# nschloe/flow

Hardware: AMD Instinct MI355X
Metric: ipcs_time_steps_per_sec (higher is better)
Workload: dtype f64

## Files before the change

flow_amd/_hip.py:

```python
import ctypes
import os

import torch

from . import device

_HERE = os.path.dirname(os.path.abspath(__file__))
LIB_PATH = os.path.join(_HERE, 'csrc', 'libflow_hip.so')

REDUCE_WORK = 4096
GMRES_MAX_RESTART = 30
GMRES_PARTIALS = (GMRES_MAX_RESTART + 2) * 1024
GMRES_STATE = 1280
SPMV_ROWS_PER_BLOCK = 256
SPMV_NNZ_PER_BLOCK = 1022
PMG_NNZ_PER_BLOCK = 2044

c_double_p = ctypes.c_void_p
c_int_p = ctypes.c_void_p


class Operator(ctypes.Structure):
    _fields_ = [
        ('kind', ctypes.c_int),
# ... 270 lines not shown

class MomentumJvp(ctypes.Structure):
    _fields_ = [
        ('mesh', ctypes.POINTER(MeshS)),
        ('W', ctypes.POINTER(SpaceS)),
        ('bfmask', ctypes.c_void_p),
        ('ui', ctypes.c_void_p),
        ('prm', NsParams),
        ('scratch', ctypes.c_void_p),
        ('nbc', ctypes.c_int),
        ('bc_dofs', ctypes.c_void_p),
        ('bc_mask', ctypes.c_void_p),
        ]


_VP = ctypes.c_void_p
_I = ctypes.c_int
_D = ctypes.c_double
_P = ctypes.POINTER
SYMBOLS = {
    'flow_abi_version': [],
    'flow_launch_count': [_P(ctypes.c_ulonglong)],
    'flow_graph_mode': [_I, ctypes.c_longlong],
    'flow_graph_stats': [_P(ctypes.c_ulonglong)],
    'flow_xcd_tile_host': [_I, _I],
    'flow_spmv_tile_nnz': [_I],
    'flow_operator_apply': [_P(Operator), _VP, _VP, _VP],
    'flow_profile_spmv_begin': [_I, _I],
    'flow_profile_spmv_end': [_P(_D), _P(_I)],
    'flow_profile_event_overhead': [_P(_D), _VP],
    'flow_profile_marker': [_I, _VP],
    'flow_profile_stream_copy': [ctypes.c_size_t, _VP, _VP, _VP],
    'flow_profile_stream_read': [ctypes.c_size_t, _VP, _VP, _VP],
    'flow_operator_diag_inv': [_P(Operator), _VP, _VP, _VP],
    'flow_dot_host': [_I, _VP, _VP, _VP, _P(_D), _VP],
    'flow_norm_host': [_I, _VP, _I, _VP, _P(_D), _VP],
    'flow_axpby': [_I, _D, _VP, _D, _VP, _VP],
    'flow_vmul': [_I, _D, _VP, _VP, _VP, _VP],
    'flow_fill': [_I, _D, _VP, _VP],
    'flow_lincomb': [_I, _I, _P(_D), _P(_VP), _VP, _VP],
    'flow_fingerprint': [_I, _P(_VP), _P(_I), _VP, _VP, _VP],
    'flow_read_doubles': [_VP, _I, _P(_D), _VP],
    'flow_extrapolation_weights': [_I, _P(_D), _D, _I, _I, _P(_D)],
    'flow_scale_rows': [_I, _VP, _VP, _VP, _VP],
    'flow_cg_solve': [_P(Operator), _VP, _P(CoarseS), _P(MgS), _VP, _VP, _D, _D,
                      _I, _I, _I, _VP, ctypes.c_size_t, _P(_I), _P(_D), _VP],
# ... 259 lines not shown
```

flow_amd/csrc/common.h:

```cpp
#pragma once
#include <hip/hip_runtime.h>

#include <algorithm>
#include <cstdarg>
#include <cstdio>
#include <functional>
#include <vector>

#include "../../include/flow_hip.h"

namespace flow {
extern unsigned long long g_launches;
}
#undef hipLaunchKernelGGL
#define hipLaunchKernelGGL(kernelName, numBlocks, numThreads, memPerBlock,        \
                           streamId, ...)                                       \
  do {                                                                          \
    ++flow::g_launches;                                                         \
    (kernelName)<<<(numBlocks), (numThreads), (memPerBlock), (streamId)>>>(     \
        __VA_ARGS__);                                                           \
  } while (0)

namespace flow {

// ... 6 lines not shown
int ilu_check(const flow_ilu* ilu, int op_size);

int pmg_apply(const flow_pmg* M, const double* r, double* z, hipStream_t st,
              const double* stop = nullptr);
int pmg_check(const flow_pmg* M, int op_size);
int tl_apply(const flow_tl* T, const double* r, double* z, hipStream_t st,
             const double* stop = nullptr);
int tl_check(const flow_tl* T, int op_size);
int operator_apply(const flow_operator* A, const double* x, double* y,
                   hipStream_t st, const double* stop = nullptr);
int operator_size(const flow_operator* A);
int sum_partials_host(double* work, int nparts, double* host, hipStream_t st);
int check_operator(const flow_operator* A);
int fill(int n, double value, double* y, hipStream_t st);
struct NoEarly {
  __device__ __forceinline__ void operator()(int, bool) const {}
};

enum Slot {
  kGamma = 0, kAlpha, kBeta, kRes2, kB2, kRho, kOmega, kRhoNew, kTmp,
  kBreak, kTarget2, kDone, kConvIt, kIter, kNumSlots = 16
};
int read_state(const double* S, double* host, hipStream_t st);
int check_comm(const flow_comm* c, long long need);
int check_rows(const flow_rows* R);
int exchange(const flow_comm* c, int count);
int exchange_halo(const flow_comm* C, const flow_rows* R, int ncomp, int sum_count,
                  int hoff, hipStream_t st);

int gather(int nout, int nplanes, const int* ptr, const int* src,
           const double* scratch, size_t plane_stride, double* out,
           hipStream_t st, size_t out_stride = 0, int r0 = 0, int r1 = 0,
           const double* stop = nullptr, const unsigned char* idrow = nullptr,
           const double* v = nullptr, size_t v_stride = 0);
int momentum_jvp_check(const flow_momentum_jvp* J);
int momentum_jvp_apply(const flow_momentum_jvp* J, const double* v, double* out,
                       hipStream_t st, int v_stride = 0, int out_stride = 0,
                       const double* stop = nullptr,
                       const double* prm_dev = nullptr);
int momentum_jvp_params(const flow_momentum_jvp* J, double* dst, hipStream_t st);

constexpr long long kReplayAutoRows = 1500000;
struct KeyHash {
  unsigned long long h = 1469598103934665603ull;
  void bytes(const void* p, size_t n) {
    const unsigned char* c = static_cast<const unsigned char*>(p);
// ... 119 lines not shown
```

flow_amd/csrc/la_kernels.hip:

```cpp
#include <cstring>

#include "common.h"
#include "csr_stream.h"

namespace flow {

thread_local char g_error[512] = "";

void set_error(const char* fmt, ...) {
  va_list ap;
  va_start(ap, fmt);
  vsnprintf(g_error, sizeof(g_error), fmt, ap);
  va_end(ap);
}

static_assert(3 * kRedBlocks + kNumSlots <= FLOW_REDUCE_WORK, "work size");


template <bool DOT>
__global__ __launch_bounds__(kBlock) void spmv_stream_kernel(
    int n, const int* __restrict__ rowptr, const int* __restrict__ cols,
    const double* __restrict__ vals0, const double* __restrict__ vals1,
    const int* __restrict__ rowblocks, const double* __restrict__ x,
    double* __restrict__ y, double* __restrict__ dpart,
// ... 1116 lines not shown
    if (state[kDone] == 1.0) {
      *iters_host = static_cast<int>(state[kConvIt]);
      *resid_host = sqrt(res2);
      return FLOW_OK;
    }
    if (launched >= maxit) {
      *iters_host = launched;
      *resid_host = sqrt(res2);
      set_error("BiCGStab did not converge in %d iterations: |r| = %.3e > %.3e",
                launched, sqrt(res2), sqrt(state[kTarget2]));
      return FLOW_NOT_CONVERGED;
    }
  }
}

}

using namespace flow;

extern "C" const char* flow_last_error(void) { return g_error; }
extern "C" int flow_abi_version(void) { return 30; }

namespace flow {
unsigned long long g_launches = 0;
}
extern "C" int flow_launch_count(unsigned long long* count_host) {
  FLOW_REQUIRE(count_host != nullptr, "flow_launch_count argument");
  *count_host = flow::g_launches;
  return FLOW_OK;
}

extern "C" int flow_spmv_tile_nnz(int kind) {
  return (kind == 2 || kind == 4) ? kTile2 - 2 : kTile - 2;
}

extern "C" int flow_xcd_tile_host(int block, int nblocks) {
  return xcd_tile(block, nblocks);
}

extern "C" int flow_profile_spmv_begin(int rows, int max_launches) {
  SpmvProfile& pf = g_spmv_profile;
  FLOW_REQUIRE(rows > 0 && max_launches > 0 && max_launches <= 100000,
               "profile arguments");
  FLOW_REQUIRE(pf.ev == nullptr, "a profile is already running");
  pf.ev = new hipEvent_t[2 * static_cast<size_t>(max_launches)];
  for (int i = 0; i < 2 * max_launches; ++i)
// ... 729 lines not shown
  const double snj = dj > 0.0 ? et / dj : 0.0;
  const double resid = fabs(snj * g[j]);
  store_scalar(S + kRes2, resid);
  store_scalar(S + kConvIt, static_cast<double>(j + 1));
  const bool done = resid <= target && !lucky;
  if (done || lucky || last) {
    const int nc = j + 1;
    col[j] = dj;
    g[j] = csj * g[j];
    for (int i = nc - 1; i >= 0; --i) {
      double t = g[i];
      for (int c = i + 1; c < nc; ++c) t -= Hs[c * ld + i] * y[c];
      const double rii = Hs[i * ld + i];
      y[i] = rii != 0.0 ? t / rii : 0.0;
    }
    for (int k = 0; k < nc; ++k) store_scalar(G + kGYc + k, y[k] / nrm[k]);
    if (done) store_scalar(S + kDone, 1.0);
    if (lucky) store_scalar(S + kDone, 3.0);
  }
}

__global__ __launch_bounds__(kBlock) void gmres_begin_kernel(
    int nparts, int have_b2, int first, int accept10, double rtol, double atol,
    const double* __restrict__ partial, double* __restrict__ S) {
  double r = 0.0, b = 0.0;
  for (int i = threadIdx.x; i < nparts; i += kBlock) {
    r += load_scalar(partial + i);
    if (have_b2) b += load_scalar(partial + kRedBlocks + i);
  }
  r = block_sum(r);
  b = block_sum(b);
  if (threadIdx.x != 0) return;
  double target;
  if (first) {
    const double b2 = have_b2 ? b : r;
    target = fmax(rtol * sqrt(b2), atol);
    store_scalar(S + kB2, b2);
    store_scalar(S + kTarget2, target);
    if (have_b2 && r > b2) {
      store_scalar(S + kTmp, 1.0);
      r = b2;
    }
  } else {
    target = load_scalar(S + kTarget2);
  }
  const double beta = sqrt(r);
  store_scalar(S + kBeta, beta);
  store_scalar(S + kRes2, beta);
  store_scalar(S + kConvIt, 0.0);
  if (!(r == r))
    store_scalar(S + kDone, 2.0);
  else if (beta <= target || (accept10 && beta <= 10.0 * target))
    store_scalar(S + kDone, 4.0);
}

// ... 143 lines not shown
  hipLaunchKernelGGL(gmres_dots_kernel<NV>, dim3(gd), dim3(kBlock), 0, st, N,  \
                     w, V + static_cast<size_t>(k0) * N,                      \
                     static_cast<size_t>(N), k0 == 0 ? 1 : 0,                 \
                     P + k0 * kRedBlocks, Pww, stop)
      FLOW_NV_SWITCH(chunk, FLOW_CALL)
#undef FLOW_CALL
    }
    hipLaunchKernelGGL(gmres_step_kernel, dim3(1), dim3(kBlock), 0, st, gd, j,
                       last ? 1 : 0, beta, target, P, G, S);
    FLOW_CHECK_LAUNCH();
    if (!last &&
        (r = gmres_combine_dev(N, j + 1, G + kGCoef, G + kGCw, w, V, w, Pnn, false,
                               stop, st)))
      return r;
    return FLOW_OK;
  };

  const bool replay = replay_wanted(N, kReplayGmres);
  KeyHash base;
  if (replay) {
    base.pod(0x676dull);
    key_operator(base, A, true);
    base.pod(dinv).obj(ilu).obj(ilu ? ilu->plan : nullptr).obj(pmg);
    base.pod(work).pod(N).pod(m);
    if (A->kind == 3) {
      jprm = G + kGJvp;
      if ((rc = momentum_jvp_params(
               static_cast<const flow_momentum_jvp*>(A->matfree), G + kGJvp, st)))
        return rc;
    }
  }
  auto arnoldi_replayed = [&](int j, bool last) -> int {
    if (!replay) return arnoldi(j, -1.0, 0.0, last);
    KeyHash key = base;
    key.pod(j).pod(last);
    hipGraphExec_t graph = nullptr;
    int nodes = 0, r;
    if ((r = replay_prepare(key.h, kReplayGmres, st,
                            [&]() { return arnoldi(j, -1.0, 0.0, last); }, &graph,
                            &nodes)))
      return r;
    return graph ? replay_launch(graph, nodes, st) : arnoldi(j, -1.0, 0.0, last);
  };

  if ((rc = fill(kNumSlots, 0.0, S, st))) return rc;
  double resid = 0.0;
  int it = 0;
  bool first = true;
  bool claimed = false;
  double state[kNumSlots];
  while (true) {
    const bool b_is_r0 = x_is_zero && it == 0;
    if (b_is_r0) {
      hipLaunchKernelGGL(axpby_kernel, dim3(gv), dim3(kBlock), 0, st, N, 1.0, b,
                         0.0, V);
    } else {
      if ((rc = apply(A, x, iwork, st))) return rc;
      hipLaunchKernelGGL(residual_kernel, dim3(gv), dim3(kBlock), 0, st, N, b,
                         iwork,
                         static_cast<const double*>(nullptr), V,
                         static_cast<double*>(nullptr));
    }
    const int have_b2 = first && !b_is_r0;
    if ((rc = dots(N, have_b2 ? 2 : 1, V, V, b, b, V, V, partial, &np, st)))
      return rc;
    hipLaunchKernelGGL(gmres_begin_kernel, dim3(1), dim3(kBlock), 0, st, np,
                       have_b2, first ? 1 : 0, claimed ? 1 : 0, rtol, atol,
                       partial, S);
    if (have_b2)
      hipLaunchKernelGGL(gmres_drop_start_kernel, dim3(gv), dim3(kBlock), 0, st,
                         N, S, b, V, x);
    FLOW_CHECK_LAUNCH();
    first = false;
    claimed = false;
    if (it >= maxit) {
      if ((rc = read_state(S, state, st))) return rc;
      resid = state[kBeta];
      if (state[kDone] == 4.0) break;
      *iters_host = it;
      *resid_host = resid;
      if (state[kDone] == 2.0) {
        set_error("GMRES broke down (NaN residual) at iteration %d", it);
      } else {
        set_error("GMRES did not converge in %d iterations: |r| = %.3e > %.3e",
                  it, resid, state[kTarget2]);
      }
      return FLOW_NOT_CONVERGED;
    }

    const int it0 = it;
    int enq = 0, cols = 0;
// ... 8 lines not shown
        const bool last = enq + 1 >= m || it0 + enq + 1 >= maxit;
        if ((rc = arnoldi_replayed(enq, last))) return rc;
      }
      if ((rc = read_state(S, state, st))) return rc;
      cols = static_cast<int>(state[kConvIt]);
      if (state[kDone] == 2.0) {
        *iters_host = it0 + cols;
        *resid_host = state[kRes2];
        set_error("GMRES broke down (NaN) at iteration %d", it0 + cols);
        return FLOW_NOT_CONVERGED;
      }
      resid = state[kRes2];
      if (state[kDone] == 4.0) {
        start_passes = true;
        break;
      }
      if (state[kDone] != 0.0) {
        converged = state[kDone] == 1.0;
        break;
      }
    }
    if (start_passes) break;
    it = it0 + (cols > 0 ? cols : 1);
    if ((rc = fill(1, 0.0, S + kDone, st))) return rc;
    if (cols > 0 &&
        (rc = gmres_combine_dev(N, cols, G + kGYc, nullptr, nullptr, Zbase, x,
                                nullptr, true, nullptr, st)))
      return rc;
    x_is_zero = 0;
    if (converged && !verify) break;
    claimed = converged;
  }
  *iters_host = it;
  *resid_host = resid;
  return FLOW_OK;
}

static int check_solver_args(const flow_operator* A, const double* b,
                             const double* x, double rtol, double atol,
                             int maxit, int check_every, int first_check,
                             const double* work, size_t work_len, size_t nvec,
                             const int* iters_host, const double* resid_host) {
  int rc = check_operator(A);
  if (rc) return rc;
  FLOW_REQUIRE(b && x && work && iters_host && resid_host, "solver pointers");
  FLOW_REQUIRE(rtol >= 0.0 && atol >= 0.0 && maxit >= 0 && check_every > 0 &&
                   first_check >= 0,
// ... 1295 lines not shown
```

flow_amd/csrc/mass_kernels.hip:

```cpp
#include "common.h"
#include "csr_stream.h"
#include "csr_stream16.h"

#include <hip/hip_fp16.h>

namespace flow {

__global__ __launch_bounds__(kBlock) void mass_residual_kernel(
    const int* __restrict__ rowptr, const int* __restrict__ cols,
    const double* __restrict__ vals, const int* __restrict__ rowblocks,
    const double* __restrict__ x, const double* __restrict__ b,
    const double* __restrict__ dinv, float* __restrict__ rho0,
    const double* __restrict__ stop) {
  __shared__ double prod[kTile];
  if (stopped(stop)) return;
  int r, r1;
  double bi = 0.0, di = 0.0;
  auto early = [&](int row, bool has) {
    if (has) {
      bi = b[row];
      di = dinv[row];
    }
  };
  const double s =
// ... 51 lines not shown
__device__ __forceinline__ void apply_mask(const unsigned char* mask, int n, int r,
                                           float own, float& s) {
  if (mask && !mask[r]) s = own;
}
__device__ __forceinline__ void apply_mask(const unsigned char* mask, int n, int r,
                                           float2 own, float2& s) {
  if (mask) {
    if (!mask[r]) s.x = own.x;
    if (!mask[n + r]) s.y = own.y;
  }
}
__device__ __forceinline__ float vaxpby(float a, float x, float b, float y) {
  return a * x + b * y;
}
__device__ __forceinline__ float2 vaxpby(float a, float2 x, float b, float2 y) {
  return make_float2(a * x.x + b * y.x, a * x.y + b * y.y);
}
struct XRow {
  double x0 = 0.0, x1 = 0.0, b0 = 0.0, b1 = 0.0;
};
__device__ __forceinline__ void load_xrow(XRow& q, const double* x,
                                          const double* base, int xs, int r,
                                          float) {
  q.x0 = x[r];
  if (base) q.b0 = base[r];
}
__device__ __forceinline__ void load_xrow(XRow& q, const double* x,
                                          const double* base, int xs, int r,
                                          float2) {
  q.x0 = x[r];
  q.x1 = x[xs + r];
  if (base) {
    q.b0 = base[r];
    q.b1 = base[xs + r];
  }
}
__device__ __forceinline__ double2 add_to_x(double* x, const XRow& q, int xs,
                                           int r, float z) {
  const double xn = q.x0 + static_cast<double>(z);
  x[r] = xn;
  const double y = q.b0 + xn;
  return make_double2(static_cast<double>(z) * z, y * y);
}
__device__ __forceinline__ double2 add_to_x(double* x, const XRow& q, int xs,
                                           int r, float2 z) {
  const double x0 = q.x0 + static_cast<double>(z.x);
  const double x1 = q.x1 + static_cast<double>(z.y);
  x[r] = x0;
  x[xs + r] = x1;
  const double y0 = q.b0 + x0;
  const double y1 = q.b1 + x1;
  return make_double2(static_cast<double>(z.x) * z.x + static_cast<double>(z.y) * z.y,
                      y0 * y0 + y1 * y1);
}

template <class V, int MODE, bool PACKED>
__global__ __launch_bounds__(kBlock) void mass_cheb_kernel(
    int n, const int* __restrict__ rowptr, const int* __restrict__ cols,
    const void* __restrict__ vals, const int* __restrict__ rowblocks,
    const unsigned char* __restrict__ mask, const V* __restrict__ g,
    const V* rho_in, V* rho_out, float c0, float c1, float c2,
    V* __restrict__ d_out, V* __restrict__ acc, double* __restrict__ x,
    const double* __restrict__ xbase, int xs,
    double* __restrict__ zz_part, double* __restrict__ xx_part,
    const double* __restrict__ stop, int own_lo = 0, int own_hi = 0x7fffffff) {
  __shared__ V prod[kMassTile];
  if (stopped(stop)) return;
  int r, r1;
  V own, rho_old, acc_old;
  vzero(own);
  vzero(rho_old);
  vzero(acc_old);
  XRow xr;
  auto early = [&](int row, bool has) {
    if (!has) return;
    own = g[row];
    if (MODE >= 1) {
      rho_old = rho_in[row];
      acc_old = acc[row];
    }
    if (MODE == 2) load_xrow(xr, x, xbase, xs, row, V());
  };
  V s = PACKED
            ? mass_tile_row_sum_packed<V>(rowptr,
                                          static_cast<const unsigned*>(vals), cols,
                                          rowblocks, g, prod, r, r1, early)
            : mass_tile_row_sum<V>(rowptr, cols,
                                   static_cast<const __half*>(vals), rowblocks, g,
                                   prod, r, r1, early);
  double2 dots = make_double2(0.0, 0.0);
  if (r < r1) {
    apply_mask(mask, n, r, own, s);
    if (MODE == 0) {
      const V rho = vaxpby(1.f, own, -c0, s);
      const V d = vaxpby(c1 * c0, own, c2, rho);
      rho_out[r] = rho;
      d_out[r] = d;
      acc[r] = vaxpby(c0, own, 1.f, d);
    } else {
      const V rho = vaxpby(1.f, rho_old, -1.f, s);
      const V d = vaxpby(c1, own, c2, rho);
      if (MODE == 1) {
        rho_out[r] = rho;
        d_out[r] = d;
        acc[r] = vaxpby(1.f, acc_old, 1.f, d);
      } else {
        dots = add_to_x(x, xr, xs, r, vaxpby(1.f, acc_old, 1.f, d));
        if (r < own_lo || r >= own_hi) dots = make_double2(0.0, 0.0);
      }
    }
  }
  if (MODE == 2) {
    const double zz = block_sum(dots.x);
    const double xx = block_sum(dots.y);
    if (threadIdx.x == 0) {
      zz_part[blockIdx.x] = zz;
      xx_part[blockIdx.x] = xx;
    }
  }
}

constexpr int kMassScalarBlock = 1024;
__global__ __launch_bounds__(kMassScalarBlock) void mass_scalar_kernel(
    int nparts, const double* __restrict__ zz_part,
    const double* __restrict__ xx_part, double contraction2, double rtol2,
    double atol2, double* __restrict__ S) {
  __shared__ double wsum[2][kMassScalarBlock / 64];
  if (stopped(S + kDone)) return;
  double z0 = 0.0, z1 = 0.0, x0 = 0.0, x1 = 0.0;
  int i = threadIdx.x;
// ... 94 lines not shown
  double theta, delta, sigma, rho;
  Cheb(double lo, double hi)
      : theta(0.5 * (hi + lo)), delta(0.5 * (hi - lo)), sigma(theta / delta),
        rho(1.0 / sigma) {}
  float first() const { return static_cast<float>(1.0 / theta); }
  void next(float* c1, float* c2) {
    const double rn = 1.0 / (2.0 * sigma - rho);
    *c1 = static_cast<float>(rn * rho);
    *c2 = static_cast<float>(2.0 * rn / delta);
    rho = rn;
  }
};

struct MassTiles {
  const int* rowblocks[16];
  int nblocks[16];
  int shift;
  int own_lo, own_hi;
};

template <class V, bool PACKED>
int correction(const flow_mass* M, const MassTiles& T, double* x,
               const double* xbase, double* zz_part, double* xx_part,
               const double* stop, hipStream_t st) {
  const flow_operator* A = M->A;
  const int n = A->n;
  const void* v16 = PACKED ? M->packed16 : M->vals16;
  const int* cols = PACKED ? M->cbase16 : A->cols;
  V* w = reinterpret_cast<V*>(M->work16) - T.shift;
  const size_t len = static_cast<size_t>(M->work16_rows > 0 ? M->work16_rows : n);
  V* rho0 = w;
  V* rho = rho0 + len;
  V* d[2] = {rho + len, rho + 2 * len};
  V* acc = rho + 3 * len;
  const dim3 blk(kBlock);
  Cheb ch(M->lam_min, M->lam_max);
  const float c0 = ch.first();
  float c1, c2;
  V* const none = nullptr;
  double* const nod = nullptr;
  ch.next(&c1, &c2);
  hipLaunchKernelGGL((mass_cheb_kernel<V, 0, PACKED>), dim3(T.nblocks[0]), blk, 0,
                     st, n, A->rowptr, cols, v16, T.rowblocks[0], A->rowmask, rho0,
                     rho0, rho, c0, c1, c2, d[0], acc, nod, nod, n, nod, nod, stop,
                     0, 0x7fffffff);
  const int products = M->steps - 1;
  for (int j = 1; j + 1 < products; ++j) {
    ch.next(&c1, &c2);
    hipLaunchKernelGGL((mass_cheb_kernel<V, 1, PACKED>), dim3(T.nblocks[j]), blk,
                       0, st, n, A->rowptr, cols, v16, T.rowblocks[j], A->rowmask,
                       d[(j - 1) & 1], rho, rho, 0.f, c1, c2, d[j & 1], acc, nod,
                       nod, n, nod, nod, stop, 0, 0x7fffffff);
  }
  ch.next(&c1, &c2);
  hipLaunchKernelGGL((mass_cheb_kernel<V, 2, PACKED>),
                     dim3(T.nblocks[products - 1]), blk, 0, st, n, A->rowptr, cols,
                     v16, T.rowblocks[products - 1], A->rowmask,
                     d[(products - 2) & 1], rho, none, 0.f, c1, c2, none, acc, x,
                     xbase, n, zz_part, xx_part, stop, T.own_lo, T.own_hi);
  FLOW_CHECK_LAUNCH();
  return FLOW_OK;
}

static MassTiles default_tiles(const flow_mass* M) {
  MassTiles T;
  for (int j = 0; j < 16; ++j) {
    T.rowblocks[j] = M->rowblocks16;
    T.nblocks[j] = M->nblocks16;
  }
  T.shift = 0;
  T.own_lo = 0;
  T.own_hi = 0x7fffffff;
  return T;
}

}

static int mass_check(const flow_mass* M) {
  FLOW_REQUIRE(M != nullptr && M->A != nullptr, "flow_mass is NULL");
  int rc = check_operator(M->A);
  if (rc) return rc;
  FLOW_REQUIRE(M->A->kind == 0 || M->A->kind == 4,
               "flow_mass: operator kind 0 (scalar) or 4 (one plane, two "
               "components)");
  FLOW_REQUIRE(M->dinv && M->rowblocks16 && (M->vals16 || M->packed16) &&
                   M->work16 && M->nblocks16 > 0,
               "flow_mass pointers");
  FLOW_REQUIRE(reinterpret_cast<uintptr_t>(M->vals16) % 16 == 0 &&
                   reinterpret_cast<uintptr_t>(M->packed16) % 16 == 0 &&
                   reinterpret_cast<uintptr_t>(M->A->cols) % 16 == 0 &&
                   reinterpret_cast<uintptr_t>(M->work16) % 16 == 0,
               "flow_mass: vals16 / packed16, cols and work16 must be 16-byte "
               "aligned");
  FLOW_REQUIRE(M->packed16 == nullptr || M->cbase16 != nullptr,
               "flow_mass: the packed stream needs the tiles' base columns");
  FLOW_REQUIRE(M->lam_max > M->lam_min && M->lam_min > 0.0,
               "Chebyshev interval (0 < lam_min < lam_max)");
  FLOW_REQUIRE(M->steps >= 3 && M->steps <= 16, "Chebyshev steps (3..16)");
  FLOW_REQUIRE(M->contraction > 0.0 && M->contraction <= 1.0,
               "contraction bound in (0, 1]");
  return FLOW_OK;
}

static int mass_solve(const flow_mass* M, const double* b, double* x,
                      const double* xbase, bool x_is_zero, double rtol,
                      double atol, int maxit, int first_check, double* work,
                      int* iters_host, double* resid_host, hipStream_t st) {
  const flow_operator* A = M->A;
  double* S = work + 3 * kRedBlocks;
  double* zz_part = work + FLOW_REDUCE_WORK;
  double* xx_part = zz_part + M->nblocks16;
  const double* stop = S + kDone;
  const double c2 = M->contraction * M->contraction;
  int rc;
  if ((rc = fill(kNumSlots, 0.0, S, st))) return rc;
  auto one = [&]() -> int {
    if (x_is_zero) {
      hipLaunchKernelGGL(mass_rho0_kernel, dim3(grid_for(A->n)), dim3(kBlock), 0,
                         st, A->n, A->kind == 4 ? 2 : 1, b, M->dinv, M->work16,
                         stop);
      x_is_zero = false;
    } else if (A->kind == 4) {
      hipLaunchKernelGGL(mass_residual_pair_kernel, dim3(A->nblocks), dim3(kBlock),
                         0, st, A->n, A->rowptr, A->cols, A->vals[0], A->rowblocks,
                         A->rowmask, x, A->n, b, M->dinv,
                         reinterpret_cast<float2*>(M->work16), stop);
    } else {
      hipLaunchKernelGGL(mass_residual_kernel, dim3(A->nblocks), dim3(kBlock), 0, st,
                         A->rowptr, A->cols, A->vals[0], A->rowblocks, x, b, M->dinv,
                         M->work16, stop);
    }
    const MassTiles T = default_tiles(M);
    if (A->kind == 4) {
      rc = M->packed16 ? correction<float2, true>(M, T, x, xbase, zz_part, xx_part,
                                                  stop, st)
                       : correction<float2, false>(M, T, x, xbase, zz_part,
                                                   xx_part, stop, st);
    } else {
      rc = M->packed16 ? correction<float, true>(M, T, x, xbase, zz_part, xx_part,
                                                 stop, st)
                       : correction<float, false>(M, T, x, xbase, zz_part, xx_part,
                                                  stop, st);
    }
    if (rc) return rc;
    hipLaunchKernelGGL(mass_scalar_kernel, dim3(1), dim3(kMassScalarBlock), 0, st,
                       M->nblocks16, zz_part, xx_part, c2, rtol * rtol, atol * atol,
                       S);
    FLOW_CHECK_LAUNCH();
    return FLOW_OK;
  };
  const bool replay = replay_wanted(A->n, kReplayMass);
  KeyHash base;
  if (replay) {
    base.pod(0x6d73ull);
    key_operator(base, A);
    base.obj(M).pod(b).pod(x).pod(xbase).pod(work).pod(rtol).pod(atol);
  }
  auto one_replayed = [&]() -> int {
    if (!replay) return one();
    KeyHash key = base;
    key.pod(x_is_zero);
    hipGraphExec_t graph = nullptr;
    int nodes = 0, r;
    const bool was_zero = x_is_zero;
    if ((r = replay_prepare(key.h, kReplayMass, st, one, &graph, &nodes))) return r;
    x_is_zero = was_zero;
    if (!graph) return one();
    x_is_zero = false;
    return replay_launch(graph, nodes, st);
  };
  double state[kNumSlots];
  int launched = 0;
  while (true) {
    const int batch = (launched == 0 && first_check > 0) ? first_check : 1;
    const int todo = (maxit - launched < batch) ? maxit - launched : batch;
    for (int k = 0; k < todo; ++k)
      if ((rc = one_replayed())) return rc;
    launched += todo;
    if ((rc = read_state(S, state, st))) return rc;
    const double zz = state[kRes2];
    if (state[kDone] == 2.0 || !(zz == zz)) {
      *iters_host = static_cast<int>(state[kConvIt]);
      *resid_host = zz;
      set_error("mass solve broke down (NaN) at correction %d", *iters_host);
      return FLOW_NOT_CONVERGED;
    }
    if (state[kDone] == 1.0) {
      *iters_host = static_cast<int>(state[kConvIt]);
      *resid_host = sqrt(zz);
      return FLOW_OK;
    }
    if (state[kDone] == 3.0) {
      *iters_host = static_cast<int>(state[kConvIt]);
      *resid_host = sqrt(zz);
      set_error("mass solve: correction %d contracted by %.3f (no "
                "contraction; the vouched bound is %.3f: not the mass matrix "
                "of straight P1/P2 triangles?)", *iters_host, state[kTmp],
                M->contraction);
      return FLOW_NOT_CONVERGED;
    }
// ... 136 lines not shown
                         dim3(kBlock), 0, st, A->n, ncomp, b, M->dinv, rho0, stop,
                         R->r0, R->r1);
    } else if (A->kind == 4) {
      hipLaunchKernelGGL(mass_residual_pair_kernel, dim3(A->nblocks), dim3(kBlock),
                         0, st, A->n, A->rowptr, A->cols, A->vals[0], A->rowblocks,
                         A->rowmask, x, A->n, b, M->dinv,
                         reinterpret_cast<float2*>(rho0), stop);
    } else {
      hipLaunchKernelGGL(mass_residual_kernel, dim3(A->nblocks), dim3(kBlock), 0, st,
                         A->rowptr, A->cols, A->vals[0], A->rowblocks, x, b, M->dinv,
                         rho0, stop);
    }
    hipLaunchKernelGGL(shard_mass_pack_kernel, dim3(gp), dim3(kMassPackBlock), 0,
                       st, *R, ncomp, k == 0 ? 1 : 0, nlast, zz_part, xx_part, rho0,
                       C->buf, stop);
    FLOW_CHECK_LAUNCH();
    (void)count;
    if ((rc = exchange_halo(C, R, ncomp, 4, 4, st))) return rc;
    hipLaunchKernelGGL(shard_mass_unpack_kernel, dim3(gs), dim3(kBlock), 0, st, *R,
                       ncomp, k == 0 ? 1 : 0, k, c2, rtol * rtol, atol * atol,
                       C->buf, rho0, S);
    FLOW_CHECK_LAUNCH();
    if (A->kind == 4)
      rc = correction<float2, false>(M, T, x, xbase, zz_part, xx_part, stop, st);
    else
      rc = correction<float, false>(M, T, x, xbase, zz_part, xx_part, stop, st);
    ++k;
    return rc;
  };
  double state[kNumSlots];
  bool started = false;
  while (true) {
    int todo = (!started && first_check > 0) ? first_check + 1 : 1;
    if (!started && first_check == 0) todo = 2;
    started = true;
    if (k + todo > maxit + 1) todo = maxit + 1 - k;
    for (int i = 0; i < todo; ++i)
      if ((rc = one())) return rc;
    if ((rc = read_state(S, state, st))) return rc;
    const double zz = state[kRes2];
    if (state[kDone] == 2.0 || !(zz == zz)) {
      *iters_host = static_cast<int>(state[kConvIt]);
      *resid_host = zz;
      set_error("sharded mass solve broke down (NaN) at correction %d",
                *iters_host);
      return FLOW_NOT_CONVERGED;
    }
    if (state[kDone] == 1.0) {
      *iters_host = static_cast<int>(state[kConvIt]);
// ... 70 lines not shown
  for (int i = blockIdx.x * blockDim.x + threadIdx.x; i < n;
       i += gridDim.x * blockDim.x)
    y[i] = b ? a[i] + b[i] : a[i];
}

extern "C" int flow_mass_solve_increment(const flow_mass* M, const double* g,
                                         const double* xbase,
                                         const double* delta0, double* x,
                                         double rtol, double atol, int maxit,
                                         int first_check, double* work,
                                         size_t work_len, int* iters_host,
                                         double* resid_host, void* stream) {
  int rc = mass_check(M);
  if (rc) return rc;
  FLOW_REQUIRE(g && xbase && x && work && iters_host && resid_host,
               "solver pointers");
  FLOW_REQUIRE(rtol >= 0.0 && atol >= 0.0 && maxit >= 1 && first_check >= 0,
               "solver tolerances");
  const size_t N = M->A->kind == 4 ? 2 * static_cast<size_t>(M->A->n) : M->A->n;
  const size_t head = FLOW_REDUCE_WORK + 2 * static_cast<size_t>(M->nblocks16);
  FLOW_REQUIRE(work_len >= head + (head & 1) + N, "mass solve workspace too small");
  hipStream_t st = as_stream(stream);
  double* delta = work + head + (head & 1);
  if (delta0) {
    hipLaunchKernelGGL(mass_sum_kernel, dim3(grid_for(N)), dim3(kBlock), 0, st,
                       static_cast<int>(N), delta0, static_cast<const double*>(nullptr),
                       delta);
    FLOW_CHECK_LAUNCH();
  } else if ((rc = fill(static_cast<int>(N), 0.0, delta, st))) {
    return rc;
  }
  rc = mass_solve(M, g, delta, xbase, delta0 == nullptr, rtol, atol, maxit,
                  first_check, work, iters_host, resid_host, st);
  hipLaunchKernelGGL(mass_sum_kernel, dim3(grid_for(N)), dim3(kBlock), 0, st,
                     static_cast<int>(N), xbase, delta, x);
  FLOW_CHECK_LAUNCH();
  return rc;
}

__global__ void mass_sum_rows_kernel(int n, int ncomp, int lo, int hi,
                                     const double* __restrict__ a,
                                     const double* __restrict__ b,
                                     double* __restrict__ y) {
  const int m = hi - lo;
  for (int t = blockIdx.x * blockDim.x + threadIdx.x; t < ncomp * m;
       t += gridDim.x * blockDim.x) {
// ... 65 lines not shown
```

flow_amd/csrc/pmg_kernels.hip:

```cpp
#include "common.h"
#include "csr_stream16.h"

#include <hip/hip_fp16.h>

namespace flow {

constexpr int kPmgQuads = 2;
constexpr int kPmgTile = kBlock * 4 * kPmgQuads;
static_assert(FLOW_PMG_NNZ_PER_BLOCK == kPmgTile - 4,
              "tile minus alignment slack (base aligned down to a multiple of 4)");
static_assert(kPmgTile == kMassTile, "one tile shape for both fp16 streams");

__device__ __forceinline__ float2 f2(float a, float b) { return make_float2(a, b); }

struct Half2x4 {
  __half2 v[4];
};
static_assert(sizeof(Half2x4) == 16, "packed quad");

template <bool C16, class Early>
__device__ __forceinline__ float2 pmg_tile_row_sum(
    const int* __restrict__ rowptr, const void* __restrict__ cols_any,
    const int* __restrict__ cbase,
    const __half2* __restrict__ vals, const int* __restrict__ rowblocks,
// ... 137 lines not shown
  }
  acc.x += own.x + d.x + extra.x;
  acc.y += own.y + d.y + extra.y;
  double zx = acc.x, zy = acc.y;
  if (bc) {
    if (bc[r]) zx = rin[r];
    if (bc[n + r]) zy = rin[static_cast<size_t>(zs) + r];
  }
  z[r] = zx;
  if (zs) z[static_cast<size_t>(zs) + r] = zy;
}

__global__ __launch_bounds__(kBlock) void pmg_init_kernel(
    int n, int rs, const double* __restrict__ r, const float2* __restrict__ dinv,
    float inv_theta, float2* __restrict__ rho0, float2* __restrict__ rho,
    float2* __restrict__ d, const double* __restrict__ stop) {
  if (stopped(stop)) return;
  for (int i = blockIdx.x * blockDim.x + threadIdx.x; i < n;
       i += gridDim.x * blockDim.x) {
    const float2 di = dinv[i];
    const float2 v = f2(static_cast<float>(r[i]) * di.x,
                        static_cast<float>(r[static_cast<size_t>(rs) + i]) * di.y);
    rho0[i] = v;
    rho[i] = v;
    d[i] = f2(inv_theta * v.x, inv_theta * v.y);
  }
}

__global__ __launch_bounds__(kBlock) void pmg_restrict_kernel(
    int n1, const int* __restrict__ rptr, const int* __restrict__ rsrc,
    const float2* __restrict__ res, const float2* __restrict__ dinv_c,
    const unsigned char* __restrict__ bcc, float inv_theta_c,
    float2* __restrict__ rhoc, float2* __restrict__ dc, float2* __restrict__ xc,
    const double* __restrict__ stop) {
  if (stopped(stop)) return;
  constexpr int kAhead = 8;
  for (int v = blockIdx.x * blockDim.x + threadIdx.x; v < n1;
       v += gridDim.x * blockDim.x) {
    const int a = rptr[v], b = rptr[v + 1];
    int idx[kAhead];
#pragma unroll
    for (int k = 0; k < kAhead; ++k) idx[k] = rsrc[a + k < b ? a + k : a];
    float2 t[kAhead];
#pragma unroll
    for (int k = 0; k < kAhead; ++k) t[k] = res[idx[k]];
    float2 s = t[0];
    float2 e = f2(0.f, 0.f);
// ... 310 lines not shown
              const double* stop) {
  const flow_pmg_level* F = &M->fine;
  const flow_pmg_level* C = &M->coarse;
  const int n = F->n, n1 = C->n;
  float2* w = reinterpret_cast<float2*>(M->work);
  float2* rho0 = w;
  float2* rho = rho0 + n;
  float2* d[3] = {rho + n, rho + 2 * static_cast<size_t>(n),
                  rho + 3 * static_cast<size_t>(n)};
  float2* x = rho + 4 * static_cast<size_t>(n);
  float2* crho = x + n;
  float2* cd[2] = {crho + n1, crho + 2 * static_cast<size_t>(n1)};
  float2* cx = crho + 3 * static_cast<size_t>(n1);
  const float2* fdiag = reinterpret_cast<const float2*>(F->diag);
  const float2* fdinv = reinterpret_cast<const float2*>(F->dinv);
  const float2* cdinv = reinterpret_cast<const float2*>(C->dinv);
  float2* const none = nullptr;
  double* const nod = nullptr;
  const unsigned char* const nob = nullptr;
  float c1, c2;

  Cheb pre(F->lam_min, F->lam_max);
  const int zs = M->scalar ? 0 : n;
  hipLaunchKernelGGL(pmg_init_kernel, dim3(grid_for(n)), dim3(kBlock), 0, st, n, zs,
                     r, fdinv, pre.first(), rho0, rho, d[0], stop);
  for (int j = 1; j < M->pre; ++j) {
    pre.next(&c1, &c2);
    launch_cheb<1>(F, d[j - 1], rho, rho, d[j - 1], c1, c2, d[j], none, none, nod,
                   nob, nod, stop, st);
  }
  launch_cheb<0>(F, d[M->pre - 1], rho, rho, fdiag, 0.f, 0.f, none, none, none, nod,
                 nob, nod, stop, st);
  Cheb co(C->lam_min, C->lam_max);
  hipLaunchKernelGGL(pmg_restrict_kernel, dim3(grid_for(n1)), dim3(kBlock), 0, st,
                     n1, M->rptr, M->rsrc, rho, cdinv, M->bc_coarse, co.first(),
                     crho, cd[0], cx, stop);
  for (int j = 1; j < M->coarse_steps; ++j) {
    co.next(&c1, &c2);
    float2* dn = cd[j & 1];
    const float2* dc = cd[(j - 1) & 1];
    launch_cheb<1>(C, dc, crho, crho, dc, c1, c2, dn, cx, none, nod, nob, nod,
                   stop, st);
  }
  hipLaunchKernelGGL(pmg_prolong_kernel, dim3(grid_for(n)), dim3(kBlock), 0, st, n,
                     reinterpret_cast<const int2*>(M->ends), d[0],
                     M->pre > 1 ? d[1] : none, M->pre > 2 ? d[2] : none, cx, x,
                     stop);
  Cheb post(F->lam_min, F->lam_max);
  if (M->post == 1) {
    launch_cheb<2>(F, x, rho0, none, none, 0.f, post.first(), none, x, none, z,
                   M->bc_fine, r, stop, st, zs);
  } else {
    launch_cheb<1>(F, x, rho0, rho, none, 0.f, post.first(), d[0], none, none, nod,
                   nob, nod, stop, st);
    for (int j = 1; j < M->post; ++j) {
// ... 145 lines not shown
```

include/flow_hip.h:

```cpp
#ifndef FLOW_HIP_H
#define FLOW_HIP_H

#include <stddef.h>

#ifdef __cplusplus
extern "C" {
#endif

#define FLOW_OK 0
#define FLOW_NOT_CONVERGED 1
#define FLOW_INVALID 2
#define FLOW_HIP_ERROR 3

#define FLOW_SPMV_ROWS_PER_BLOCK 256
#define FLOW_SPMV_NNZ_PER_BLOCK 1022
int flow_spmv_tile_nnz(int kind);

const char* flow_last_error(void);
int flow_abi_version(void);
int flow_launch_count(unsigned long long* count_host);
int flow_graph_mode(int mode, long long auto_rows);
int flow_graph_stats(unsigned long long* stats_host);
int flow_xcd_tile_host(int block, int nblocks);

typedef struct {
  int kind;
  int n;
  int nnz;
  int nblocks;
  const int* rowptr;
  const int* cols;
  const int* rowblocks;
  const double* vals[4];
  const void* matfree;
  const unsigned char* rowmask;
} flow_operator;

int flow_operator_apply(const flow_operator* A, const double* x, double* y,
                        void* stream);
int flow_operator_diag_inv(const flow_operator* A, const int* diag_idx,
                           double* dinv, void* stream);

int flow_profile_spmv_begin(int rows, int max_launches);
int flow_profile_spmv_end(double* total_us, int* launches);
// ... 570 lines not shown
```

profiles/summarize.py:

```python
from __future__ import print_function

import csv
import glob
import json
import os
import sys
from collections import defaultdict


def _marker_window(directory, steps=None):
    t = {1: None, 2: None}
    once_per_step = []
    for path in _find(directory, 'kernel_trace.csv'):
        with open(path) as fh:
            for r in csv.DictReader(fh):
                name = r['Kernel_Name']
                if 'profile_marker_kernel' in name:
                    g = int(r['Grid_Size_X']) // max(int(r.get(
                        'Workgroup_Size_X', 64) or 64), 1)
                    if g in t:
                        if t[g] is None:
                            t[g] = int(r['Start_Timestamp'])
                elif 'pressure_rhs_kernel' in name:
                    once_per_step.append(int(r['Start_Timestamp']))
# ... 210 lines not shown
    run_name, run_count, run_us = None, 0, 0.0
    end = ev[0][0]

    def flush():
        if run_name is not None:
            lines.append('%5d x %-60s %9.1f us' % (run_count, run_name[:60], run_us))
    for s0, e0, name in ev:
        gap = (s0 - end) * 1e-3
        if gap >= min_gap_us:
            flush()
            run_name, run_count, run_us = None, 0, 0.0
            lines.append('        ---- idle %.0f us ----' % gap)
        if name != run_name:
            flush()
            run_name, run_count, run_us = name, 0, 0.0
        run_count += 1
        run_us += (e0 - s0) * 1e-3
        end = max(end, e0)
    flush()
    with open(out, 'w') as fh:
        fh.write('\n'.join(lines) + '\n')


if __name__ == '__main__':
    if sys.argv[1] == 'counters':
        counters(sys.argv[2], *sys.argv[3:])
        sys.exit(0)
    if sys.argv[1] == 'gaps':
        gaps(sys.argv[2], sys.argv[3],
             window=sys.argv[4] if len(sys.argv) > 4 else None)
    elif sys.argv[1] == 'sequence':
        sequence(sys.argv[2], sys.argv[3], sys.argv[4])
    elif sys.argv[1] == 'stats':
        stats(sys.argv[2], sys.argv[3],
              window=sys.argv[4] if len(sys.argv) > 4 else None)
    else:
        pmc(*sys.argv[2:7])
```

Baseline: 127.1.

## Fold auxiliary copy, fill and sum passes into neighbouring kernels

Adds a default-on pass_fusion switch. With it on, GMRES clears its state slots inside gmres_begin_kernel instead of issuing separate fill launches. The mass solve reads its initial guess from delta0 and writes x = xbase + delta directly from the correction kernel, which removes the separate mass_sum_kernel passes. The PMG init kernel no longer copies rho0 into rho, and the first Chebyshev step reads rho0 instead. Together these cut small kernel launches and redundant memory traffic per time step, at the cost of more conditional paths and aliasing assumptions.

```diff
diff --git a/flow_amd/_hip.py b/flow_amd/_hip.py
--- a/flow_amd/_hip.py
+++ b/flow_amd/_hip.py
@@ -316,6 +316,7 @@
     'flow_abi_version': [],
     'flow_launch_count': [_P(ctypes.c_ulonglong)],
     'flow_graph_mode': [_I, ctypes.c_longlong],
+    'flow_pass_fusion': [_I],
     'flow_graph_stats': [_P(ctypes.c_ulonglong)],
     'flow_xcd_tile_host': [_I, _I],
     'flow_spmv_tile_nnz': [_I],
diff --git a/flow_amd/csrc/common.h b/flow_amd/csrc/common.h
--- a/flow_amd/csrc/common.h
+++ b/flow_amd/csrc/common.h
@@ -52,6 +52,7 @@
   kBreak, kTarget2, kDone, kConvIt, kIter, kNumSlots = 16
 };
 int read_state(const double* S, double* host, hipStream_t st);
+bool pass_fusion();
 int check_comm(const flow_comm* c, long long need);
 int check_rows(const flow_rows* R);
 int exchange(const flow_comm* c, int count);
diff --git a/flow_amd/csrc/la_kernels.hip b/flow_amd/csrc/la_kernels.hip
--- a/flow_amd/csrc/la_kernels.hip
+++ b/flow_amd/csrc/la_kernels.hip
@@ -1162,6 +1162,16 @@
 extern "C" int flow_abi_version(void) { return 30; }
 
 namespace flow {
+static bool g_pass_fusion = true;
+bool pass_fusion() { return g_pass_fusion; }
+}
+extern "C" int flow_pass_fusion(int enable) {
+  const int was = flow::g_pass_fusion ? 1 : 0;
+  if (enable >= 0) flow::g_pass_fusion = enable != 0;
+  return was;
+}
+
+namespace flow {
 unsigned long long g_launches = 0;
 }
 extern "C" int flow_launch_count(unsigned long long* count_host) {
@@ -1937,7 +1947,7 @@
 
 __global__ __launch_bounds__(kBlock) void gmres_begin_kernel(
     int nparts, int have_b2, int first, int accept10, double rtol, double atol,
-    const double* __restrict__ partial, double* __restrict__ S) {
+    const double* __restrict__ partial, double* __restrict__ S, int reset = 0) {
   double r = 0.0, b = 0.0;
   for (int i = threadIdx.x; i < nparts; i += kBlock) {
     r += load_scalar(partial + i);
@@ -1946,6 +1956,10 @@
   r = block_sum(r);
   b = block_sum(b);
   if (threadIdx.x != 0) return;
+  if (reset == 2)
+    for (int i = 0; i < kNumSlots; ++i) store_scalar(S + i, 0.0);
+  else if (reset == 1)
+    store_scalar(S + kDone, 0.0);
   double target;
   if (first) {
     const double b2 = have_b2 ? b : r;
@@ -2135,7 +2149,7 @@
     base.pod(0x676dull);
     key_operator(base, A, true);
     base.pod(dinv).obj(ilu).obj(ilu ? ilu->plan : nullptr).obj(pmg);
-    base.pod(work).pod(N).pod(m);
+    base.pod(work).pod(N).pod(m).pod(pass_fusion());
     if (A->kind == 3) {
       jprm = G + kGJvp;
       if ((rc = momentum_jvp_params(
@@ -2156,7 +2170,8 @@
     return graph ? replay_launch(graph, nodes, st) : arnoldi(j, -1.0, 0.0, last);
   };
 
-  if ((rc = fill(kNumSlots, 0.0, S, st))) return rc;
+  const bool fused = pass_fusion();
+  if (!fused && (rc = fill(kNumSlots, 0.0, S, st))) return rc;
   double resid = 0.0;
   int it = 0;
   bool first = true;
@@ -2179,7 +2194,7 @@
       return rc;
     hipLaunchKernelGGL(gmres_begin_kernel, dim3(1), dim3(kBlock), 0, st, np,
                        have_b2, first ? 1 : 0, claimed ? 1 : 0, rtol, atol,
-                       partial, S);
+                       partial, S, fused ? (first ? 2 : 1) : 0);
     if (have_b2)
       hipLaunchKernelGGL(gmres_drop_start_kernel, dim3(gv), dim3(kBlock), 0, st,
                          N, S, b, V, x);
@@ -2234,7 +2249,7 @@
     }
     if (start_passes) break;
     it = it0 + (cols > 0 ? cols : 1);
-    if ((rc = fill(1, 0.0, S + kDone, st))) return rc;
+    if (!fused && (rc = fill(1, 0.0, S + kDone, st))) return rc;
     if (cols > 0 &&
         (rc = gmres_combine_dev(N, cols, G + kGYc, nullptr, nullptr, Zbase, x,
                                 nullptr, true, nullptr, st)))
diff --git a/flow_amd/csrc/mass_kernels.hip b/flow_amd/csrc/mass_kernels.hip
--- a/flow_amd/csrc/mass_kernels.hip
+++ b/flow_amd/csrc/mass_kernels.hip
@@ -97,34 +97,43 @@
 __device__ __forceinline__ void load_xrow(XRow& q, const double* x,
                                           const double* base, int xs, int r,
                                           float) {
-  q.x0 = x[r];
+  if (x) q.x0 = x[r];
   if (base) q.b0 = base[r];
 }
 __device__ __forceinline__ void load_xrow(XRow& q, const double* x,
                                           const double* base, int xs, int r,
                                           float2) {
-  q.x0 = x[r];
-  q.x1 = x[xs + r];
+  if (x) {
+    q.x0 = x[r];
+    q.x1 = x[xs + r];
+  }
   if (base) {
     q.b0 = base[r];
     q.b1 = base[xs + r];
   }
 }
-__device__ __forceinline__ double2 add_to_x(double* x, const XRow& q, int xs,
-                                           int r, float z) {
+__device__ __forceinline__ double2 add_to_x(double* x, double* yout,
+                                           const XRow& q, int xs, int r,
+                                           float z) {
   const double xn = q.x0 + static_cast<double>(z);
   x[r] = xn;
   const double y = q.b0 + xn;
+  if (yout) yout[r] = y;
   return make_double2(static_cast<double>(z) * z, y * y);
 }
-__device__ __forceinline__ double2 add_to_x(double* x, const XRow& q, int xs,
-                                           int r, float2 z) {
+__device__ __forceinline__ double2 add_to_x(double* x, double* yout,
+                                           const XRow& q, int xs, int r,
+                                           float2 z) {
   const double x0 = q.x0 + static_cast<double>(z.x);
   const double x1 = q.x1 + static_cast<double>(z.y);
   x[r] = x0;
   x[xs + r] = x1;
   const double y0 = q.b0 + x0;
   const double y1 = q.b1 + x1;
+  if (yout) {
+    yout[r] = y0;
+    yout[xs + r] = y1;
+  }
   return make_double2(static_cast<double>(z.x) * z.x + static_cast<double>(z.y) * z.y,
                       y0 * y0 + y1 * y1);
 }
@@ -135,10 +144,11 @@
     const void* __restrict__ vals, const int* __restrict__ rowblocks,
     const unsigned char* __restrict__ mask, const V* __restrict__ g,
     const V* rho_in, V* rho_out, float c0, float c1, float c2,
-    V* __restrict__ d_out, V* __restrict__ acc, double* __restrict__ x,
+    V* __restrict__ d_out, V* __restrict__ acc, double* x,
     const double* __restrict__ xbase, int xs,
     double* __restrict__ zz_part, double* __restrict__ xx_part,
-    const double* __restrict__ stop, int own_lo = 0, int own_hi = 0x7fffffff) {
+    const double* __restrict__ stop, int own_lo = 0, int own_hi = 0x7fffffff,
+    const double* xin = nullptr, double* __restrict__ yout = nullptr) {
   __shared__ V prod[kMassTile];
   if (stopped(stop)) return;
   int r, r1;
@@ -154,7 +164,7 @@
       rho_old = rho_in[row];
       acc_old = acc[row];
     }
-    if (MODE == 2) load_xrow(xr, x, xbase, xs, row, V());
+    if (MODE == 2) load_xrow(xr, xin, xbase, xs, row, V());
   };
   V s = PACKED
             ? mass_tile_row_sum_packed<V>(rowptr,
@@ -180,7 +190,7 @@
         d_out[r] = d;
         acc[r] = vaxpby(1.f, acc_old, 1.f, d);
       } else {
-        dots = add_to_x(x, xr, xs, r, vaxpby(1.f, acc_old, 1.f, d));
+        dots = add_to_x(x, yout, xr, xs, r, vaxpby(1.f, acc_old, 1.f, d));
         if (r < own_lo || r >= own_hi) dots = make_double2(0.0, 0.0);
       }
     }
@@ -321,7 +331,8 @@
 template <class V, bool PACKED>
 int correction(const flow_mass* M, const MassTiles& T, double* x,
                const double* xbase, double* zz_part, double* xx_part,
-               const double* stop, hipStream_t st) {
+               const double* stop, hipStream_t st, const double* xin,
+               double* yout = nullptr) {
   const flow_operator* A = M->A;
   const int n = A->n;
   const void* v16 = PACKED ? M->packed16 : M->vals16;
@@ -356,7 +367,8 @@
                      dim3(T.nblocks[products - 1]), blk, 0, st, n, A->rowptr, cols,
                      v16, T.rowblocks[products - 1], A->rowmask,
                      d[(products - 2) & 1], rho, none, 0.f, c1, c2, none, acc, x,
-                     xbase, n, zz_part, xx_part, stop, T.own_lo, T.own_hi);
+                     xbase, n, zz_part, xx_part, stop, T.own_lo, T.own_hi, xin,
+                     yout);
   FLOW_CHECK_LAUNCH();
   return FLOW_OK;
 }
@@ -401,10 +413,16 @@
   return FLOW_OK;
 }
 
+struct MassStart {
+  bool apart = false;
+  const double* x0 = nullptr;
+};
 static int mass_solve(const flow_mass* M, const double* b, double* x,
                       const double* xbase, bool x_is_zero, double rtol,
                       double atol, int maxit, int first_check, double* work,
-                      int* iters_host, double* resid_host, hipStream_t st) {
+                      int* iters_host, double* resid_host, hipStream_t st,
+                      MassStart start = MassStart(), double* yout = nullptr,
+                      int* enqueued = nullptr) {
   const flow_operator* A = M->A;
   double* S = work + 3 * kRedBlocks;
   double* zz_part = work + FLOW_REDUCE_WORK;
@@ -412,34 +430,37 @@
   const double* stop = S + kDone;
   const double c2 = M->contraction * M->contraction;
   int rc;
+  if (enqueued) *enqueued = 0;
   if ((rc = fill(kNumSlots, 0.0, S, st))) return rc;
+  bool first = true;
   auto one = [&]() -> int {
-    if (x_is_zero) {
+    const double* xin = (first && start.apart) ? start.x0 : x;
+    if (x_is_zero && first) {
       hipLaunchKernelGGL(mass_rho0_kernel, dim3(grid_for(A->n)), dim3(kBlock), 0,
                          st, A->n, A->kind == 4 ? 2 : 1, b, M->dinv, M->work16,
                          stop);
-      x_is_zero = false;
     } else if (A->kind == 4) {
       hipLaunchKernelGGL(mass_residual_pair_kernel, dim3(A->nblocks), dim3(kBlock),
                          0, st, A->n, A->rowptr, A->cols, A->vals[0], A->rowblocks,
-                         A->rowmask, x, A->n, b, M->dinv,
+                         A->rowmask, xin, A->n, b, M->dinv,
                          reinterpret_cast<float2*>(M->work16), stop);
     } else {
       hipLaunchKernelGGL(mass_residual_kernel, dim3(A->nblocks), dim3(kBlock), 0, st,
-                         A->rowptr, A->cols, A->vals[0], A->rowblocks, x, b, M->dinv,
-                         M->work16, stop);
-    }
+                         A->rowptr, A->cols, A->vals[0], A->rowblocks, xin, b,
+                         M->dinv, M->work16, stop);
+    }
+    first = false;
     const MassTiles T = default_tiles(M);
     if (A->kind == 4) {
       rc = M->packed16 ? correction<float2, true>(M, T, x, xbase, zz_part, xx_part,
-                                                  stop, st)
+                                                  stop, st, xin, yout)
                        : correction<float2, false>(M, T, x, xbase, zz_part,
-                                                   xx_part, stop, st);
+                                                   xx_part, stop, st, xin, yout);
     } else {
       rc = M->packed16 ? correction<float, true>(M, T, x, xbase, zz_part, xx_part,
-                                                 stop, st)
+                                                 stop, st, xin, yout)
                        : correction<float, false>(M, T, x, xbase, zz_part, xx_part,
-                                                  stop, st);
+                                                  stop, st, xin, yout);
     }
     if (rc) return rc;
     hipLaunchKernelGGL(mass_scalar_kernel, dim3(1), dim3(kMassScalarBlock), 0, st,
@@ -454,18 +475,19 @@
     base.pod(0x6d73ull);
     key_operator(base, A);
     base.obj(M).pod(b).pod(x).pod(xbase).pod(work).pod(rtol).pod(atol);
+    base.pod(start.apart).pod(start.x0).pod(yout);
   }
   auto one_replayed = [&]() -> int {
     if (!replay) return one();
     KeyHash key = base;
-    key.pod(x_is_zero);
+    key.pod(x_is_zero && first).pod(start.apart && first);
     hipGraphExec_t graph = nullptr;
     int nodes = 0, r;
-    const bool was_zero = x_is_zero;
+    const bool was_first = first;
     if ((r = replay_prepare(key.h, kReplayMass, st, one, &graph, &nodes))) return r;
-    x_is_zero = was_zero;
+    first = was_first;
     if (!graph) return one();
-    x_is_zero = false;
+    first = false;
     return replay_launch(graph, nodes, st);
   };
   double state[kNumSlots];
@@ -473,8 +495,10 @@
   while (true) {
     const int batch = (launched == 0 && first_check > 0) ? first_check : 1;
     const int todo = (maxit - launched < batch) ? maxit - launched : batch;
-    for (int k = 0; k < todo; ++k)
+    for (int k = 0; k < todo; ++k) {
       if ((rc = one_replayed())) return rc;
+      if (enqueued) ++*enqueued;
+    }
     launched += todo;
     if ((rc = read_state(S, state, st))) return rc;
     const double zz = state[kRes2];
@@ -657,9 +681,10 @@
                        C->buf, rho0, S);
     FLOW_CHECK_LAUNCH();
     if (A->kind == 4)
-      rc = correction<float2, false>(M, T, x, xbase, zz_part, xx_part, stop, st);
+      rc = correction<float2, false>(M, T, x, xbase, zz_part, xx_part, stop, st,
+                                     x);
     else
-      rc = correction<float, false>(M, T, x, xbase, zz_part, xx_part, stop, st);
+      rc = correction<float, false>(M, T, x, xbase, zz_part, xx_part, stop, st, x);
     ++k;
     return rc;
   };
@@ -776,6 +801,24 @@
   FLOW_REQUIRE(work_len >= head + (head & 1) + N, "mass solve workspace too small");
   hipStream_t st = as_stream(stream);
   double* delta = work + head + (head & 1);
+  auto apart = [&](const double* v) {
+    return v == nullptr || v + N <= x || x + N <= v;
+  };
+  if (pass_fusion() && apart(xbase) && apart(g) && apart(delta0)) {
+    MassStart start;
+    start.apart = true;
+    start.x0 = delta0;
+    int enqueued = 0;
+    rc = mass_solve(M, g, delta, xbase, delta0 == nullptr, rtol, atol, maxit,
+                    first_check, work, iters_host, resid_host, st, start, x,
+                    &enqueued);
+    if (enqueued == 0) {
+      hipLaunchKernelGGL(mass_sum_kernel, dim3(grid_for(N)), dim3(kBlock), 0, st,
+                         static_cast<int>(N), xbase, delta0, x);
+      FLOW_CHECK_LAUNCH();
+    }
+    return rc;
+  }
   if (delta0) {
     hipLaunchKernelGGL(mass_sum_kernel, dim3(grid_for(N)), dim3(kBlock), 0, st,
                        static_cast<int>(N), delta0, static_cast<const double*>(nullptr),
diff --git a/flow_amd/csrc/pmg_kernels.hip b/flow_amd/csrc/pmg_kernels.hip
--- a/flow_amd/csrc/pmg_kernels.hip
+++ b/flow_amd/csrc/pmg_kernels.hip
@@ -183,7 +183,7 @@
     const float2 v = f2(static_cast<float>(r[i]) * di.x,
                         static_cast<float>(r[static_cast<size_t>(rs) + i]) * di.y);
     rho0[i] = v;
-    rho[i] = v;
+    if (rho) rho[i] = v;
     d[i] = f2(inv_theta * v.x, inv_theta * v.y);
   }
 }
@@ -540,15 +540,17 @@
 
   Cheb pre(F->lam_min, F->lam_max);
   const int zs = M->scalar ? 0 : n;
+  const bool fused = pass_fusion();
   hipLaunchKernelGGL(pmg_init_kernel, dim3(grid_for(n)), dim3(kBlock), 0, st, n, zs,
-                     r, fdinv, pre.first(), rho0, rho, d[0], stop);
+                     r, fdinv, pre.first(), rho0, fused ? none : rho, d[0], stop);
+  const float2* rho_first = fused ? rho0 : rho;
   for (int j = 1; j < M->pre; ++j) {
     pre.next(&c1, &c2);
-    launch_cheb<1>(F, d[j - 1], rho, rho, d[j - 1], c1, c2, d[j], none, none, nod,
-                   nob, nod, stop, st);
-  }
-  launch_cheb<0>(F, d[M->pre - 1], rho, rho, fdiag, 0.f, 0.f, none, none, none, nod,
-                 nob, nod, stop, st);
+    launch_cheb<1>(F, d[j - 1], j == 1 ? rho_first : rho, rho, d[j - 1], c1, c2,
+                   d[j], none, none, nod, nob, nod, stop, st);
+  }
+  launch_cheb<0>(F, d[M->pre - 1], M->pre == 1 ? rho_first : rho, rho, fdiag, 0.f,
+                 0.f, none, none, none, nod, nob, nod, stop, st);
   Cheb co(C->lam_min, C->lam_max);
   hipLaunchKernelGGL(pmg_restrict_kernel, dim3(grid_for(n1)), dim3(kBlock), 0, st,
                      n1, M->rptr, M->rsrc, rho, cdinv, M->bc_coarse, co.first(),
diff --git a/include/flow_hip.h b/include/flow_hip.h
--- a/include/flow_hip.h
+++ b/include/flow_hip.h
@@ -20,6 +20,7 @@
 int flow_abi_version(void);
 int flow_launch_count(unsigned long long* count_host);
 int flow_graph_mode(int mode, long long auto_rows);
+int flow_pass_fusion(int enable);
 int flow_graph_stats(unsigned long long* stats_host);
 int flow_xcd_tile_host(int block, int nblocks);
 
diff --git a/profiles/summarize.py b/profiles/summarize.py
--- a/profiles/summarize.py
+++ b/profiles/summarize.py
@@ -256,7 +256,43 @@
         fh.write('\n'.join(lines) + '\n')
 
 
+def neighbours(directory, out, window, kernels):
+    ev = []
+    for path in _find(directory, 'kernel_trace.csv'):
+        with open(path) as fh:
+            for r in csv.DictReader(fh):
+                ev.append((int(r['Start_Timestamp']), int(r['End_Timestamp']),
+                           r['Kernel_Name'].split('(')[0].replace('void ', '')
+                           .replace('flow::', ''), int(r['Grid_Size_X'])))
+    ev.sort()
+    lo, hi = _window(directory, window, ev[-1][1])
+    ev = [e for e in ev if hi >= e[0] >= lo
+          and 'profile_marker_kernel' not in e[2]]
+    wanted = kernels.split(',')
+    rows = defaultdict(lambda: [0, 0.0])
+    for i, (s0, e0, name, grid) in enumerate(ev):
+        if not any(w in name for w in wanted):
+            continue
+        before = ev[i - 1][2] if i > 0 else '(window start)'
+        after = ev[i + 1][2] if i + 1 < len(ev) else '(window end)'
+        key = (name, grid, before, after)
+        rows[key][0] += 1
+        rows[key][1] += (e0 - s0) * 1e-3
+    lines = ['| kernel | grid | before | after | launches | total us |',
+             '|---|---|---|---|---|---|']
+    for (name, grid, before, after), (cnt, us) in sorted(
+            rows.items(), key=lambda kv: (kv[0][0], -kv[1][1])):
+        lines.append('| %s | %d | %s | %s | %d | %.1f |' % (
+            name, grid, before, after, cnt, us))
+    with open(out, 'w') as fh:
+        fh.write('\n'.join(lines) + '\n')
+    print('\n'.join(lines[:60]))
+
+
 if __name__ == '__main__':
+    if sys.argv[1] == 'neighbours':
+        neighbours(*sys.argv[2:6])
+        sys.exit(0)
     if sys.argv[1] == 'counters':
         counters(sys.argv[2], *sys.argv[3:])
         sys.exit(0)
```

Result: no change. 127.7, median of 6 (+0.5%).
